# luigifreda/plvs

Measured on AMD Instinct MI355X. Metric: Mvoxels/sec TSDF integrate (chisel 5 cm / 5 m, 640x480 RGB-D), higher is better.
Workload: dtype f32; 1 GPU; configs[2] stand-in, STREAMING: see DESIGN.md 4.1 / 4.6; mode=order-free (fixed-point sums; sdf / weight within tolerance), longest_voxel_run=25008, parallelism=chunk-hash shard x1

## Files before the change

### plvs_amd/csrc/tsdf_walk.hpp

```cpp
#pragma once
#include <hip/hip_runtime.h>

#include <cstdint>

#include "tsdf_chisel_core.hpp"
#include "tsdf_directory.hpp"
#include "tsdf_tiles.hpp"
#include "tsdf_walk_table.hpp"

namespace {

using namespace plvs::chisel;
using plvs::tsdf::cloud_of;
using plvs::tsdf::tile_span;
using plvs::tsdf::tile_span_tables;
using plvs::tsdf::TileSpan;
using plvs::tsdf::kCoordBias;
using plvs::tsdf::kErrCoordRange;
using plvs::tsdf::kErrDirectoryMiss;
using plvs::tsdf::kErrPoolFull;
using plvs::tsdf::home_bucket;
using plvs::tsdf::next_bucket;

constexpr int kWalkRays = 512;
constexpr int kMaskWords = kWalkRays / 32;
#ifndef PLVS_WALK_ENTRIES
#define PLVS_WALK_ENTRIES 4096
#endif
constexpr int kWalkEntries = PLVS_WALK_ENTRIES;
constexpr int kWalkLimit = kWalkEntries * 7 / 8;
constexpr int kWalkWindow = kWalkLimit / 2;
constexpr int kWalkChunks = 64;
constexpr uint32_t kErrScratch = 8u;

#ifdef PLVS_WALK_PROF
__device__ unsigned long long g_walk_prof[16];
__device__ unsigned long long g_apply_items[8192][4];
#define WALK_PROF_BEGIN()                                         \
  long long prof_t = (long long)clock64();                        \
  unsigned long long prof_acc[9] = {0, 0, 0, 0, 0, 0, 0, 0, 0}
#define WALK_PROF(k)                                               \
  do {                                                             \
    const long long now = (long long)clock64();                    \
    prof_acc[k] += (unsigned long long)(now - prof_t);             \
    prof_t = now;                                                  \
  } while (0)
#define WALK_PROF_END()                                            \
  do {                                                             \
    if (threadIdx.x == 0)                                          \
      for (int k = 0; k < 9; ++k) atomicAdd(&g_walk_prof[k], prof_acc[k]); \
  } while (0)
#else
#define WALK_PROF_BEGIN() do {} while (0)
#define WALK_PROF(k) do {} while (0)
#define WALK_PROF_END() do {} while (0)
#endif

struct WalkCounters {
  unsigned long long total_visits;
  uint32_t err;
  uint32_t num_heads;
  uint32_t num_updated;
  uint32_t max_run;
  uint32_t num_desc;
  uint32_t run_need;
  uint32_t rec_top, seg_top;
  uint32_t ncold;
  uint32_t split_tiles;
  uint32_t num_parts;
  uint32_t num_multi;
  uint32_t ndeferred;
  uint32_t ndeferred2;
  uint32_t over_small;
  uint32_t skip;
  uint32_t collect_top;
  uint32_t collect_parts;
  uint32_t ndeferred3;
};

constexpr int kLogLen = 16;
constexpr int kSlabs = 8;
constexpr int kSlabVox = kChunkVox / kSlabs;

struct SubTile {
  uint16_t lo, hi;
  uint32_t vlo, vhi;
  int32_t cloud;
};

constexpr uint32_t kKeyEmpty = 0xFFFFFFFFu;
constexpr int kBuckets = kWalkEntries / 4;
constexpr int kOriginBias = 512;

constexpr int log2_of(int v) { return v <= 1 ? 0 : 1 + log2_of(v / 2); }
struct WalkShared {
  static constexpr int kEntries = kWalkEntries, kBucketCount = kWalkEntries / 4, kLogLen = ::kLogLen;
  alignas(16) uint32_t ekey[kWalkEntries];
  int32_t org[3];
  uint32_t cand[kWalkRays / 64];
  int32_t worg[kWalkRays / 64][3];
  uint32_t run_total, vis_total;
  uint32_t ccode[kWalkChunks];
  int32_t cslot[kWalkChunks];
  uint32_t ccnt[kWalkChunks * kSlabs];
  uint16_t cbase[kWalkChunks * kSlabs];
  uint32_t rbase;
  SubTile stack[16];
  int sp;
  uint32_t nent;
  uint32_t overflow;
  uint32_t wsum[kWalkRays / 64];
  uint32_t next, nrays;
};
template <int E>
struct FastShared {
  static constexpr int kEntries = E, kBucketCount = E / 4, kLogLen = E == 1536 ? ::kLogLen - 1 : ::kLogLen;
  static_assert(E % kWalkRays == 0 && E >= 1024, "every thread owns E / kWalkRays entries (and a bucket four)");
  alignas(16) uint32_t ekey[E];
  uint32_t cand[kWalkRays / 64];
  int32_t worg[kWalkRays / 64][3];
  uint32_t run_total, vis_total;
  uint32_t ccode[kWalkChunks];
  int32_t cslot[kWalkChunks];
  uint32_t ccnt[kWalkChunks * kSlabs];
  uint16_t cbase[kWalkChunks * kSlabs];
  uint32_t rcnt[kWalkChunks * kSlabs];
  uint16_t rcbase[kWalkChunks * kSlabs];
  uint32_t any_cold;
  uint32_t nent, overflow;
};


__device__ __forceinline__ bool rel_key(int vx, int vy, int vz, int ox, int oy, int oz, uint32_t* key) {
  const uint32_t dx = (uint32_t)(vx - ox), dy = (uint32_t)(vy - oy), dz = (uint32_t)(vz - oz);
  *key = dx | (dy << 10) | (dz << 20);
  return ((dx | dy | dz) >> 10) == 0u;
}
__device__ __forceinline__ int origin_of(int v) { return (v - kOriginBias) & ~15; }
constexpr uint32_t kChunkCodeMask = 0x3F0FC3F0u;
__device__ __forceinline__ uint32_t chunk_code(uint32_t key) { return key & kChunkCodeMask; }
__device__ __forceinline__ uint32_t voxel_in_chunk(uint32_t key) {
  return (key & 15u) | ((key >> 6) & 0xF0u) | ((key >> 12) & 0xF00u);
}
__device__ __forceinline__ void chunk_of_code(uint32_t code, int ox, int oy, int oz, int* cx, int* cy, int* cz) {
  *cx = (ox >> 4) + (int)((code >> 4) & 63u);
  *cy = (oy >> 4) + (int)((code >> 14) & 63u);
  *cz = (oz >> 4) + (int)((code >> 24) & 63u);
}
constexpr uint32_t kKeyMul = plvs::tsdf::kTableKeyMul, kKeyMulInv = plvs::tsdf::kTableKeyMulInv;
__device__ __forceinline__ uint32_t table_key(uint32_t key) { return key * kKeyMul; }
__device__ __forceinline__ uint32_t voxel_key(uint32_t tkey) { return tkey * kKeyMulInv; }
template <class SH>
__device__ __forceinline__ uint32_t key_bucket(uint32_t tkey) { return home_bucket<SH::kBucketCount>(tkey); }

__device__ __forceinline__ uint32_t wave_scan_incl(uint32_t x) {
  x += (uint32_t)__builtin_amdgcn_update_dpp(0, (int)x, 0x111, 0xf, 0xf, false);
  x += (uint32_t)__builtin_amdgcn_update_dpp(0, (int)x, 0x112, 0xf, 0xf, false);
  x += (uint32_t)__builtin_amdgcn_update_dpp(0, (int)x, 0x114, 0xf, 0xf, false);
  x += (uint32_t)__builtin_amdgcn_update_dpp(0, (int)x, 0x118, 0xf, 0xf, false);
  x += (uint32_t)__builtin_amdgcn_update_dpp(0, (int)x, 0x142, 0xa, 0xf, false);
  x += (uint32_t)__builtin_amdgcn_update_dpp(0, (int)x, 0x143, 0xc, 0xf, false);
  return x;
}
__device__ __forceinline__ uint32_t wave_sum(uint32_t x) {
  return (uint32_t)__builtin_amdgcn_readlane((int)wave_scan_incl(x), 63);
}

__device__ __forceinline__ int bucket_match(const uint4 k4, uint32_t want) {
  const bool c0 = k4.x == want, c1 = k4.y == want, c2 = k4.z == want, c3 = k4.w == want;
  const int j = c3 ? 3 : (c2 ? 2 : (c1 ? 1 : 0));
  return (c0 | c1 | c2 | c3) ? j : -1;
}

constexpr int kProbeCap = plvs::tsdf::kTableProbeCap;
template <class SH>
__device__ __forceinline__ int table_find_or_insert(SH& S, uint32_t key ) {
  uint32_t b = key_bucket<SH>(key);
  for (int probe = 0; probe < kProbeCap; ++probe) {
    const uint4 k4 = *reinterpret_cast<const uint4*>(&S.ekey[4 * b]);
    const int j = bucket_match(k4, key);
    if (j >= 0) return (int)(4 * b) + j;
    const int je = bucket_match(k4, kKeyEmpty);
    if (je >= 0) {
      const uint32_t old = atomicCAS(&S.ekey[4 * b + je], kKeyEmpty, key);
      if (old == kKeyEmpty || old == key) return (int)(4 * b) + je;
      continue;
    }
    b = next_bucket<SH::kBucketCount>(b);
  }
  S.overflow = 1u;
  return -1;
}
template <class SH>
__device__ __forceinline__ int table_find(const SH& S, uint32_t key) {
  uint32_t b = key_bucket<SH>(key);
  for (int probe = 0; probe < SH::kBucketCount; ++probe) {
    const int j = bucket_match(*reinterpret_cast<const uint4*>(&S.ekey[4 * b]), key);
    if (j >= 0) return (int)(4 * b) + j;
    b = next_bucket<SH::kBucketCount>(b);
  }
  return -1;
}

__device__ __forceinline__ float sqrt_rn_normal(float x) {
  const float s = __builtin_amdgcn_sqrtf(x);
  const float sm = __uint_as_float(__float_as_uint(s) - 1u), sp = __uint_as_float(__float_as_uint(s) + 1u);
  const float rm = fmaf(-sm, s, x), rp = fmaf(-sp, s, x);
  float r = (rm <= 0.0f) ? sm : s;
  r = (rp > 0.0f) ? sp : r;
  return r;
}
__device__ __forceinline__ float div_rn_normal(float a, float b) {
// ... 1 lines not shown
  const float y = fmaf(fmaf(-b, y0, 1.0f), y0, y0);
  const float q = a * y;
  return fmaf(fmaf(-q, b, a), y, q);
}
__device__ __forceinline__ float signed_dist_fast(const Pose& pose, float depth, float c0, float c1, float c2) {
  float cc[3];
  xform(pose.Ri, pose.ti, c0, c1, c2, cc);
  const float n2 = sqnorm3(cc[0], cc[1], cc[2]);
  const bool plain = !(n2 >= 0x1p-80f && n2 <= 0x1p80f) || !(fabsf(cc[2]) >= 0x1p-40f && fabsf(cc[2]) <= 0x1p40f);
  if (__builtin_expect(plain, 0)) return sqrtf(n2) * (depth / cc[2] - 1);
  return sqrt_rn_normal(n2) * (div_rn_normal(depth, cc[2]) - 1);
}
__device__ __forceinline__ float uniform_f(float x) {
  return __int_as_float(__builtin_amdgcn_readfirstlane(__float_as_int(x)));
}
struct LeanRay {
  float A[9], b[3];
  float tau_in, tau_out;
};
__device__ __forceinline__ void lean_ray(const Params& P, const Pose& pose, const Ray& ray, LeanRay* L) {
#pragma unroll
  for (int k = 0; k < 9; ++k) L->A[k] = uniform_f(pose.Ri[k] * P.resolution);
#pragma unroll
  for (int k = 0; k < 3; ++k)
    L->b[k] = uniform_f(fmaf(pose.Ri[3 * k], P.half_voxel, fmaf(pose.Ri[3 * k + 1], P.half_voxel, fmaf(pose.Ri[3 * k + 2], P.half_voxel, pose.ti[k]))));
  const float mx = (ray.start[0] + ray.end[0]) * (0.5f * P.resolution) - pose.t[0];
  const float my = (ray.start[1] + ray.end[1]) * (0.5f * P.resolution) - pose.t[1];
  const float mz = (ray.start[2] + ray.end[2]) * (0.5f * P.resolution) - pose.t[2];
  const float obl2 = fmaxf(sqnorm3(mx, my, mz) / (ray.depth * ray.depth), 1.0f);
  float ext = 0.0f;
#pragma unroll
  for (int k = 0; k < 3; ++k) ext = fmaxf(ext, fmaxf(fabsf(ray.start[k]), fabsf(ray.end[k])));
  const float m = fabsf(pose.ti[0]) + fabsf(pose.ti[1]) + fabsf(pose.ti[2]) + 3.0f * (ext + 4.0f) * P.resolution + ray.depth + 1.0f;
  const float band = m * obl2 * 0x1p-19f;
  L->tau_in = ray.truncation - band;
  L->tau_out = ray.truncation + band;
}
__device__ __forceinline__ float lean_u(const LeanRay& L, float depth, float fx, float fy, float fz) {
  const float c0 = fmaf(L.A[0], fx, fmaf(L.A[1], fy, fmaf(L.A[2], fz, L.b[0])));
  const float c1 = fmaf(L.A[3], fx, fmaf(L.A[4], fy, fmaf(L.A[5], fz, L.b[1])));
  const float c2 = fmaf(L.A[6], fx, fmaf(L.A[7], fy, fmaf(L.A[8], fz, L.b[2])));
  const float n2 = fmaf(c0, c0, fmaf(c1, c1, c2 * c2));
  return __builtin_amdgcn_sqrtf(n2) * ((depth - c2) * __builtin_amdgcn_rcpf(c2));
}
__device__ __forceinline__ bool two_tier_visit(const Params& P, const Pose& pose, const Ray& ray, const LeanRay& L, float fx,
                                               float fy, float fz, float* u) {
  *u = lean_u(L, ray.depth, fx, fy, fz);
  const float au = fabsf(*u);
  bool in = au < L.tau_in;
  if (__builtin_expect(!in && au < L.tau_out, 0)) {
    const float c0 = fx * P.resolution + P.half_voxel, c1 = fy * P.resolution + P.half_voxel,
                c2 = fz * P.resolution + P.half_voxel;
    *u = signed_dist_fast(pose, ray.depth, c0, c1, c2);
    in = fabsf(*u) < ray.truncation;
  }
  return in;
}

template <class OnVisit>
__device__ __forceinline__ uint32_t walk_one(const Params& P, const Pose& pose, const Ray& ray, uint32_t vlo,
                                             uint32_t vhi, OnVisit&& on_visit) {
  RayCursor cur;
  OwnerCache owner;
  LeanRay L;
  lean_ray(P, pose, ray, &L);
  ray_begin(ray, &cur);
  int vx, vy, vz;
  uint32_t nv = 0;
  bool go = true;
  while (go && nv < vhi && ray_next(&cur, &vx, &vy, &vz)) {
    float u = 0.0f;
    const bool ok = chunk_owned(P, vx >> 4, vy >> 4, vz >> 4, &owner) &&
                    two_tier_visit(P, pose, ray, L, (float)vx, (float)vy, (float)vz, &u);
    if (ok && nv >= vlo) go = on_visit(nv - vlo, vx, vy, vz, u);
    nv += ok ? 1u : 0u;
  }
  return nv;
}

__device__ __forceinline__ int lean_reach(const Ray& ray) {
  const float maxDist = sqnorm3(ray.end[0] - ray.start[0], ray.end[1] - ray.start[1], ray.end[2] - ray.start[2]);
  return (int)(__builtin_amdgcn_sqrtf(maxDist)) + 3;
}
template <bool kAcc, bool kRuns, bool kRayOfVp, class SH>
__device__ __forceinline__ uint32_t walk_lean(const Params& P, const Pose& pose, const Ray& ray, SH& S, int ox, int oy,
                                              int oz, int tid, float wu_scaled, uint32_t q_w, int32_t* e_wuu,
                                              unsigned long long* e_wc, uint32_t* e_last, uint16_t* vlog, uint32_t rid) {
  RayCursor cur;
  ray_begin(ray, &cur);
  if (cur.done) return 0u;
  LeanRay L;
  lean_ray(P, pose, ray, &L);
  uint32_t key = table_key((uint32_t)(cur.x - ox) | ((uint32_t)(cur.y - oy) << 10) | ((uint32_t)(cur.z - oz) << 20));
  const uint32_t endkey = table_key((uint32_t)(cur.endX - ox) | ((uint32_t)(cur.endY - oy) << 10) | ((uint32_t)(cur.endZ - oz) << 20));
  const uint32_t kx = table_key((uint32_t)cur.stepX), ky = table_key((uint32_t)cur.stepY << 10), kz = table_key((uint32_t)cur.stepZ << 20);
  float fx = (float)cur.x, fy = (float)cur.y, fz = (float)cur.z;
  const float sfx = (float)cur.stepX, sfy = (float)cur.stepY, sfz = (float)cur.stepZ;
  float tmx = cur.tMaxX, tmy = cur.tMaxY, tmz = cur.tMaxZ;
  const float tdx = cur.stepX ? cur.tDeltaX : 0.0f, tdy = cur.stepY ? cur.tDeltaY : 0.0f, tdz = cur.stepZ ? cur.tDeltaZ : 0.0f;
  static_assert(kWalkRays * sizeof(uint16_t) == 1024, "the count is the offset >> 10");
  uint32_t vp = (uint32_t)tid * (uint32_t)sizeof(uint16_t);
  for (int guard = 0; guard < kRayStepGuard; ++guard) {
    const float d = sqnorm3(fx - cur.sx, fy - cur.sy, fz - cur.sz);
    const bool stop = (d > cur.maxDist) || (key == endkey);
    float u;
    if (two_tier_visit(P, pose, ray, L, fx, fy, fz, &u)) {
      int e;
      {
        const uint32_t b = key_bucket<SH>(key);
        const uint4 k4 = *reinterpret_cast<const uint4*>(&S.ekey[4 * b]);
        const int j = bucket_match(k4, key);
        if (j >= 0) {
          e = (int)(4 * b) + j;
        } else {
          const int je = bucket_match(k4, kKeyEmpty);
          uint32_t old = 0u;
          if (je >= 0) old = atomicCAS(&S.ekey[4 * b + je], kKeyEmpty, key);
          e = (je >= 0 && (old == kKeyEmpty || old == key)) ? (int)(4 * b) + je : table_find_or_insert(S, key);
        }
      }
      if (__builtin_expect(e < 0, 0)) break;
      if (kRuns && vp < (uint32_t)(SH::kLogLen * kWalkRays * sizeof(uint16_t)))
        *reinterpret_cast<uint16_t*>(reinterpret_cast<char*>(vlog) + vp) = (uint16_t)e;
      if (kAcc) {
        atomicAdd(&e_wuu[e], __float2int_rn(wu_scaled * u));
        atomicAdd(&e_wc[e], (1ull << 32) | (unsigned long long)q_w);
        atomicMax(&e_last[e], kRayOfVp ? (vp >> 1) & (uint32_t)(kWalkRays - 1) : rid);
      }
      vp += (uint32_t)(kWalkRays * sizeof(uint16_t));
    }
    if (stop) break;
    const bool x_lt_y = tmx < tmy, x_lt_z = tmx < tmz, y_lt_z = tmy < tmz;
    const bool go_x = x_lt_y && x_lt_z, go_y = !x_lt_y && y_lt_z;
    const float mx = go_x ? 1.0f : 0.0f, my = go_y ? 1.0f : 0.0f, mz = (go_x || go_y) ? 0.0f : 1.0f;
    fx = fmaf(mx, sfx, fx);
    fy = fmaf(my, sfy, fy);
    fz = fmaf(mz, sfz, fz);
    tmx = fmaf(mx, tdx, tmx);
    tmy = fmaf(my, tdy, tmy);
    tmz = fmaf(mz, tdz, tmz);
    key += go_x ? kx : (go_y ? ky : kz);
  }
  return vp >> 10;
}

constexpr int kGridTileW = 32, kGridTileH = kWalkRays / kGridTileW;
static_assert(kGridTileW == 32 && kGridTileH == kMaskWords, "one mask word per grid row of a tile");
struct GridSrc {
  const float* depth;
  const float* cam;
  unsigned long long image_stride;
  uint32_t pitch;
  uint32_t step, gw, gh;
  uint32_t ntx, nty;
  uint32_t key_bits;
  double min_depth, max_depth;
  unsigned long long bgr_image_stride;
  uint32_t bgr_pitch;
  float inv_ntx, inv_nty;
};
struct GridTile {
  uint32_t cloud, row0, col0;
};
__device__ __forceinline__ uint32_t fast_div(uint32_t x, uint32_t d, float inv) {
  if (x >= (1u << 24)) return x / d;
  uint32_t q = (uint32_t)((float)x * inv);
  const int32_t r = (int32_t)(x - q * d);
  q = r < 0 ? q - 1u : ((uint32_t)r >= d ? q + 1u : q);
  return q;
}
__device__ __forceinline__ uint32_t grid_band(const GridSrc& g, uint32_t gtile) { return fast_div(gtile, g.ntx, g.inv_ntx); }
__device__ __forceinline__ GridTile grid_tile_of_band(const GridSrc& g, uint32_t gtile, uint32_t band) {
  const uint32_t c = fast_div(band, g.nty, g.inv_nty);
  return GridTile{c, (band - c * g.nty) * (uint32_t)kGridTileH, (gtile - band * g.ntx) * (uint32_t)kGridTileW};
}
__device__ __forceinline__ GridTile grid_tile(const GridSrc& g, uint32_t gtile) {
  return grid_tile_of_band(g, gtile, grid_band(g, gtile));
}
__device__ __forceinline__ bool grid_point(const GridSrc& g, const GridTile& t, uint32_t rid, float* x, float* y, float* z) {
  const uint32_t m = t.row0 + rid / (uint32_t)kGridTileW, n = t.col0 + rid % (uint32_t)kGridTileW;
  if (m >= g.gh || n >= g.gw) return false;
  const float d = g.depth[(size_t)t.cloud * g.image_stride + (size_t)(m * g.step) * g.pitch + n * g.step];
  if (!(((double)d > g.min_depth) && ((double)d < g.max_depth))) return false;
  const float2 c = reinterpret_cast<const float2*>(g.cam)[m * g.gw + n];
  *x = c.x * d;
  *y = c.y * d;
  *z = d;
  return true;
}
typedef float GridFloat2 __attribute__((ext_vector_type(2)));
__device__ __forceinline__ GridSrc grid_fetch(const GridSrc* __restrict__ gp) {
  GridSrc g{};
  g.depth = gp->depth; g.cam = gp->cam; g.image_stride = gp->image_stride; g.pitch = gp->pitch; g.step = gp->step;
  g.gw = gp->gw; g.gh = gp->gh; g.ntx = gp->ntx; g.nty = gp->nty; g.min_depth = gp->min_depth; g.max_depth = gp->max_depth;
  g.inv_ntx = gp->inv_ntx; g.inv_nty = gp->inv_nty;
  asm volatile("" ::"s"(g.depth), "s"(g.cam), "s"(g.image_stride), "s"(g.pitch), "s"(g.step), "s"(g.gw), "s"(g.gh), "s"(g.ntx),
               "s"(g.nty), "s"(g.min_depth), "s"(g.max_depth), "s"(g.inv_ntx), "s"(g.inv_nty));
  return g;
}
__device__ __forceinline__ bool grid_pixel_load(const GridSrc& g, const GridTile& t, uint32_t rid, float* d, GridFloat2* c) {
  const uint32_t m = t.row0 + rid / (uint32_t)kGridTileW, n = t.col0 + rid % (uint32_t)kGridTileW;
  if (m >= g.gh || n >= g.gw) return false;
  const auto* depth = (const __attribute__((address_space(1))) float*)(uintptr_t)g.depth;
  const auto* cam = (const __attribute__((address_space(1))) GridFloat2*)(uintptr_t)g.cam;
  *d = depth[(size_t)t.cloud * g.image_stride + (size_t)(m * g.step) * g.pitch + n * g.step];
  *c = cam[m * g.gw + n];
  return true;
// ... 532 lines not shown
    }
    for (uint32_t r0 = 0; fits_runs && r0 < nruns; r0 += kMaskCap) {
      __syncthreads();
#pragma unroll
      for (int k = 0; k < kMaskCap * kMaskWords / kWalkRays; ++k) raw[tid + k * kWalkRays] = 0u;
      __syncthreads();
      if (walks && nmine) {
        const uint32_t logged = min(nmine, (uint32_t)kLogLen);
        for (uint32_t k = 0; k < logged; ++k) {
          const uint32_t m = (uint32_t)e_midx[vlog[k * kWalkRays + tid]] - r0;
          if (m < (uint32_t)kMaskCap) atomicOr(&raw[m * kMaskWords + (tid >> 5)], 1u << (tid & 31));
        }
        if (nmine > (uint32_t)kLogLen) {
          walk_one(P, pose, ray, st.vlo, st.vhi, [&](uint32_t k, int vx, int vy, int vz, float) {
            if (k >= (uint32_t)kLogLen) {
              uint32_t key;
              const int e = rel_key(vx, vy, vz, fox, foy, foz, &key) ? table_find(S, table_key(key)) : -1;
              const uint32_t m = e >= 0 ? (uint32_t)e_midx[e] - r0 : 0xFFFFFFFFu;
              if (m < (uint32_t)kMaskCap) atomicOr(&raw[m * kMaskWords + (tid >> 5)], 1u << (tid & 31));
            }
            return true;
          });
        }
      }
      __syncthreads();
#pragma unroll
      for (int k = 0; k < kPer; ++k) {
        const uint32_t m = (uint32_t)e_midx[tid + k * kWalkRays];
        if (m == 0xFFFFu || m < r0 || m >= r0 + (uint32_t)kMaskCap) continue;
        const size_t d = ((size_t)tile << runs.r1_log2) + emitted + m;
        runs.dkey[d] = vkey[k];
        const uint32_t* mk = raw + (m - r0) * kMaskWords;
        uint4* dst = reinterpret_cast<uint4*>(runs.masks + d * kMaskWords);
#pragma unroll
        for (int q = 0; q < kMaskWords / 4; ++q) dst[q] = make_uint4(mk[4 * q], mk[4 * q + 1], mk[4 * q + 2], mk[4 * q + 3]);
      }
    }
    __syncthreads();
    if (tid == 0) S.run_total = emitted + nruns;
    WALK_PROF(7);
    if (single && !was_split) break;
  }

#pragma unroll
  for (int off = 32; off > 0; off >>= 1) my_visits += (uint32_t)__shfl_xor((int)my_visits, off);
  if (lane == 0 && my_visits) atomicAdd(&S.vis_total, my_visits);
  __syncthreads();
  if (tid == 0) {
    if (kRuns) runs.run_cnt[tile] = min(S.run_total, 1u << runs.r1_log2);
    if (kAcc) {
      out.tile_visits[tile] = S.vis_total;
      if (flushes == 0) out.seg_cnt[tile] = 0;
    }
    if (was_split) atomicAdd(&ctr->split_tiles, 1u);
  }
  WALK_PROF(8);
  WALK_PROF_END();
  }
}

constexpr int walk_fast_waves(int E) { return E > 2048 ? 2 : (E > 1536 ? 4 : 6); }
constexpr int kFastEntriesSmall = 1536;
template <int E, bool kGrid>
__device__ __forceinline__ void walk_fast_tile(
    const Params& P, float scale_u, float scale_w, const float* __restrict__ xyz, int npoints,
    const int32_t* __restrict__ offsets, int nclouds, const Pose* __restrict__ poses, const Directory& dir,
    int32_t* __restrict__ num_chunks, WalkCounters* __restrict__ ctr, const uint32_t* __restrict__ rgbw,
    const uint32_t* __restrict__ sat, const AccOut& out, const RunOut& runs, const TileMap& tmap, uint32_t rec_stride,
    uint32_t* __restrict__ deferred, uint32_t* __restrict__ ndeferred, const uint32_t tile, const bool listed_other,
    const GridSrc* __restrict__ grid_arg) {
  const GridSrc* __restrict__ const grid = kGrid ? grid_arg : nullptr;
  constexpr int kPer = E / kWalkRays;
  constexpr int kLimit = E * 7 / 8;
  constexpr int kMaskCapE = E / 4;
  constexpr int kLogLen = FastShared<E>::kLogLen;
  static_assert(kMaskCapE * kMaskWords % kWalkRays == 0, "the mask area is cleared by whole rounds of the tile's threads");
  __shared__ FastShared<E> S;
  __shared__ uint32_t raw[4 * E];
  __shared__ uint16_t vlog[kLogLen * kWalkRays];
  static_assert(offsetof(FastShared<E>, cbase) == offsetof(FastShared<E>, ccnt) + sizeof(S.ccnt), "cbase follows ccnt");
  constexpr bool kMidxOverlay = sizeof(S.ccnt) + sizeof(S.cbase) >= E * sizeof(uint16_t);
  __shared__ uint16_t e_midx_own[kMidxOverlay ? 1 : E];
  uint16_t* const e_midx = kMidxOverlay ? reinterpret_cast<uint16_t*>(S.ccnt) : e_midx_own;
  int32_t* const e_wuu = reinterpret_cast<int32_t*>(raw);
  unsigned long long* const e_wc = reinterpret_cast<unsigned long long*>(raw + E);
  uint32_t* const e_last = raw + 3 * E;
  const int tid = threadIdx.x, lane = tid & 63, wid = tid >> 6;
  const uint32_t gtile = tmap.tile_of(tile);
  const GridSrc gs = kGrid ? grid_fetch(grid_arg) : GridSrc{};
  const GridTile gt = kGrid ? grid_tile(gs, gtile) : GridTile{0u, 0u, 0u};
  const TileSpan span = grid ? TileSpan{(int)gt.cloud, 0u, (uint32_t)kWalkRays}
                      : tmap.tables ? tile_span_tables(offsets, nclouds, gtile, kWalkRays)
                                    : tile_span(offsets, nclouds, gtile, kWalkRays);
  const uint32_t first = span.first, nrays = span.nrays;
  const int cloud = span.cloud;
  bool defer = P.shard_count > 1 || listed_other;
  WALK_PROF_BEGIN();
  uint32_t nv = 0;
  uint32_t rid = (uint32_t)threadIdx.x;
  bool walks = false;
  int ox = 0, oy = 0, oz = 0;
  if (!defer) {
    const Pose& pose = poses[cloud];
    float gd = 0.0f, pR[9], pt[3];
    GridFloat2 gc = {0.0f, 0.0f};
    bool gin = false;
    if (kGrid) {
      gin = grid_pixel_load(gs, gt, rid, &gd, &gc);
#pragma unroll
      for (int k = 0; k < 9; ++k) pR[k] = pose.R[k];
#pragma unroll
      for (int k = 0; k < 3; ++k) pt[k] = pose.t[k];
    }
    subtile_reset(S, tid);
#pragma unroll
    for (int k = 0; k < kWalkChunks * kSlabs / kWalkRays; ++k) S.rcnt[tid + k * kWalkRays] = 0u;
#pragma unroll
    for (int k = 0; k < 4 * kPer; ++k) raw[tid + k * kWalkRays] = 0u;
    if (tid == 0) {
      S.run_total = 0;
      S.vis_total = 0;
      S.any_cold = 0;
    }
    Ray ray;
    if (kGrid) {
      asm volatile("" ::"s"(pR[0]), "s"(pR[1]), "s"(pR[2]), "s"(pR[3]), "s"(pR[4]), "s"(pR[5]), "s"(pR[6]), "s"(pR[7]), "s"(pR[8]),
                   "s"(pt[0]), "s"(pt[1]), "s"(pt[2]));
      Pose cw{};
#pragma unroll
      for (int k = 0; k < 9; ++k) cw.R[k] = pR[k];
#pragma unroll
      for (int k = 0; k < 3; ++k) cw.t[k] = pt[k];
      walks = gin && grid_depth_ok(gs, gd) && ray_of_point(P, cw, gc.x * gd, gc.y * gd, gd, &ray, &ctr->err);
    } else {
      walks = (uint32_t)tid < nrays && tile_ray_src(P, xyz, grid, gt, pose, first, rid, &ray, &ctr->err);
    }
    const float wu = walks ? P.weight / (2.0f * ray.truncation) : 0.0f;
    {
      const unsigned long long wm = __ballot(walks);
      if (lane == 0) S.cand[wid] = wm ? 1u : 0u;
      if (wm && lane == __ffsll((long long)wm) - 1)
        for (int k = 0; k < 3; ++k) S.worg[wid][k] = origin_of((int)floorf(ray.start[k]));
    }
    WALK_PROF(0);
    __syncthreads();
    WALK_PROF(1);
    {
      int w0 = 0;
#pragma unroll
      for (int w = kWalkRays / 64 - 1; w >= 0; --w) w0 = S.cand[w] ? w : w0;
      ox = S.worg[w0][0]; oy = S.worg[w0][1]; oz = S.worg[w0][2];
      uint32_t anyc = 0;
#pragma unroll
      for (int w = 0; w < kWalkRays / 64; ++w) anyc |= S.cand[w];
      if (anyc == 0u) {
        if (tid == 0) {
          out.seg_cnt[tile] = 0;
          runs.run_cnt[tile] = 0;
          out.tile_visits[tile] = 0;
        }
        return;
      }
    }
    bool fits = false;
    if (walks) {
      const int reach = lean_reach(ray);
      const int rx = (int)floorf(ray.start[0]) - ox, ry = (int)floorf(ray.start[1]) - oy, rz = (int)floorf(ray.start[2]) - oz;
      fits = min(min(rx, ry), rz) - reach >= 0 && max(max(rx, ry), rz) + reach <= 1023;
      if (!fits) S.overflow = 1u;
    }
    if (fits) {
      nv = walk_lean<true, true, true>(P, pose, ray, S, ox, oy, oz, tid, wu * scale_u, (uint32_t)__float2int_rn(wu * scale_w), e_wuu,
                                 e_wc, e_last, vlog, rid);
    }
  }
  uint32_t ekey[kPer];
  WALK_PROF(2);
  if (!defer) {
    __syncthreads();
    WALK_PROF(3);
#pragma unroll
    for (int k = 0; k < kPer; ++k) {
      ekey[k] = S.ekey[tid + k * kWalkRays];
      if (ekey[k] != kKeyEmpty) ekey[k] = voxel_key(ekey[k]);
    }
    uint32_t wave_n = 0;
#pragma unroll
    for (int k = 0; k < kPer; ++k) wave_n += (uint32_t)__popcll(__ballot(ekey[k] != kKeyEmpty));
    if (lane == 0 && wave_n) atomicAdd(&S.nent, wave_n);
  } else {
#pragma unroll
    for (int k = 0; k < kPer; ++k) ekey[k] = kKeyEmpty;
  }
  int ci[kPer];
  uint32_t rank[kPer], rrank[kPer], vkey[kPer], elast[kPer];
  unsigned long long ewc[kPer];
  uint32_t need = 0;
  bool multi = false;
#pragma unroll
  for (int k = 0; k < kPer; ++k) {
    ci[k] = -2;
    rank[k] = 0;
    rrank[k] = 0;
    vkey[k] = 0xFFFFFFFFu;
    elast[k] = 0;
    ewc[k] = 0;
  }
  if (!defer) {
#pragma unroll
    for (int k = 0; k < kPer; ++k) {
      if (ekey[k] == kKeyEmpty) continue;
      bool won;
      ci[k] = chunk_cache_insert(S, chunk_code(ekey[k]), &won);
      if (ci[k] < 0) {
        S.overflow = 1u;
        continue;
      }
      int slot = S.cslot[ci[k]];
      if (slot < 0) {
        int cx, cy, cz;
        chunk_of_code(chunk_code(ekey[k]), ox, oy, oz, &cx, &cy, &cz);
        slot = dir_find_or_insert_hit(dir, cx, cy, cz, num_chunks, &ctr->err);
        if (slot >= 0) S.cslot[ci[k]] = slot;
      }
      if (slot < 0) continue;
      vkey[k] = (uint32_t)slot * (uint32_t)kChunkVox + voxel_in_chunk(ekey[k]);
    }
    uint32_t cw[kPer];
#pragma unroll
    for (int k = 0; k < kPer; ++k) {
      cw[k] = 0u;
      if (vkey[k] != 0xFFFFFFFFu) cw[k] = sat ? sat[vkey[k] >> 5] : rgbw[vkey[k]];
    }
#pragma unroll
    for (int k = 0; k < kPer; ++k) {
      if (vkey[k] == 0xFFFFFFFFu) continue;
      const uint32_t vid = vkey[k] % (uint32_t)kChunkVox;
      ewc[k] = e_wc[tid + k * kWalkRays];
      elast[k] = e_last[tid + k * kWalkRays];
      rank[k] = atomicAdd(&S.ccnt[ci[k] * kSlabs + (int)(vid / kSlabVox)], 1u);
    }
#pragma unroll
    for (int k = 0; k < kPer; ++k) {
      if (vkey[k] == 0xFFFFFFFFu) continue;
      const bool cold = sat ? ((cw[k] >> (vkey[k] & 31u)) & 1u) == 0u : (cw[k] >> 24) < 254u;
      if (cold) {
        need |= 1u << k;
        multi = multi || (uint32_t)(ewc[k] >> 32) > 1u;
        rrank[k] = atomicAdd(&S.rcnt[ci[k] * kSlabs + (int)((vkey[k] % (uint32_t)kChunkVox) / kSlabVox)], 1u);
      }
    }
  }
  WALK_PROF(4);
  if (need) S.any_cold = 1u;
  const bool any_multi = __syncthreads_or(multi ? 1 : 0) != 0;
  const bool any_cold = S.any_cold != 0u;
  WALK_PROF(5);
  const bool too_many = !defer && S.nent > (uint32_t)kLimit;
  if (E == 2048 && tid == 0 && !defer && S.nent > (uint32_t)(kFastEntriesSmall * 7 / 8)) atomicAdd(&ctr->over_small, 1u);
  if (!defer) defer = S.overflow != 0 || too_many;
  if (defer) {
    if (tid == 0) {
      out.seg_cnt[tile] = 0;
      runs.run_cnt[tile] = 0;
      out.tile_visits[tile] = 0;
      deferred[atomicAdd(ndeferred, 1u)] = tile | (too_many ? 0x80000000u : 0u);
    }
    return;
  }
  {
    const uint32_t v = wave_sum(nv);
    if (lane == 0 && v) atomicAdd(&S.vis_total, v);
  }
  const uint32_t rbase = tile * rec_stride;
  uint32_t nruns;
  uint32_t ticket = 0, ticket_sg = 0xFFFFFFFFu;
  {
    uint32_t sub[kSlabs], c = 0, rsub[kSlabs], rc = 0;
#pragma unroll
    for (int s = 0; s < kSlabs; ++s) {
      sub[s] = c;
      c += S.ccnt[lane * kSlabs + s];
      rsub[s] = 0;
    }
    uint32_t rinc = 0;
    nruns = 0;
    if (any_cold) {
#pragma unroll
      for (int s = 0; s < kSlabs; ++s) {
        rsub[s] = rc;
        rc += S.rcnt[lane * kSlabs + s];
      }
      rinc = wave_scan_incl(rc);
      nruns = (uint32_t)__builtin_amdgcn_readlane((int)rinc, 63);
#pragma unroll
      for (int s = 0; s < kSlabs; ++s) S.rcbase[lane * kSlabs + s] = (uint16_t)(rinc - rc + rsub[s]);
    }
    const uint32_t both = wave_scan_incl(c | (c ? 1u << 16 : 0u));
    const uint32_t inc = both & 0xFFFFu, sinc = both >> 16;
#pragma unroll
    for (int s = 0; s < kSlabs; ++s) S.cbase[lane * kSlabs + s] = (uint16_t)(inc - c + sub[s]);
    if (wid == 0) {
      const uint32_t stot = (uint32_t)__builtin_amdgcn_readlane((int)sinc, 63);
      if (lane == 0) out.seg_cnt[tile] = stot;
      if (c) {
        const uint32_t sg = tile * (uint32_t)kWalkChunks + sinc - 1u;
        if (out.chunk_nseg) {
          ticket = atomicAdd(&out.chunk_nseg[S.cslot[lane]], 1u);
          ticket_sg = sg;
        }
        out.seg[2 * (size_t)sg] = make_uint4((uint32_t)S.cslot[lane], rbase + inc - c, c, gtile);
        out.seg[2 * (size_t)sg + 1] = pack_suboffsets(sub);
        if (runs.rseg) {
          runs.rseg[2 * (size_t)sg] = make_uint4((tile << runs.r1_log2) + rinc - rc, rc, 0u, 0u);
          runs.rseg[2 * (size_t)sg + 1] = pack_suboffsets(rsub);
        }
      }
    }
  }
#pragma unroll
  for (int k = 0; k < kPer; ++k) {
    if (vkey[k] == 0xFFFFFFFFu) continue;
    const uint32_t vid = vkey[k] % (uint32_t)kChunkVox;
    const uint4 r = make_uint4(vid | ((uint32_t)(ewc[k] >> 32) << 12),
                               grid ? grid_order_key(*grid, gt, elast[k]) : first + elast[k],
                               (uint32_t)e_wuu[tid + k * kWalkRays], (uint32_t)ewc[k]);
    out.rec[rbase + S.cbase[ci[k] * kSlabs + (int)(vid / kSlabVox)] + rank[k]] = r;
  }
  WALK_PROF(6);
  const bool fits_runs = nruns <= (1u << runs.r1_log2);
  if (!fits_runs && tid == 0) {
    atomicOr(&ctr->err, kErrScratch);
    atomicMax(&ctr->run_need, nruns);
  }
  uint32_t mrun[kPer];
#pragma unroll
  for (int k = 0; k < kPer; ++k)
    mrun[k] = (need & (1u << k)) ? (uint32_t)S.rcbase[ci[k] * kSlabs + (int)((vkey[k] % (uint32_t)kChunkVox) / kSlabVox)] + rrank[k] : 0xFFFFu;
  if (!any_multi) {
#pragma unroll
    for (int k = 0; k < kPer; ++k) {
      if (!(need & (1u << k)) || !fits_runs) continue;
      const size_t d = ((size_t)tile << runs.r1_log2) + mrun[k];
      runs.dkey[d] = vkey[k];
      uint4* dst = reinterpret_cast<uint4*>(runs.masks + d * kMaskWords);
      const uint32_t word = elast[k] >> 5, bit = 1u << (elast[k] & 31u);
#pragma unroll
      for (int q = 0; q < kMaskWords / 4; ++q)
        dst[q] = make_uint4(word == 4u * q ? bit : 0u, word == 4u * q + 1u ? bit : 0u, word == 4u * q + 2u ? bit : 0u,
                            word == 4u * q + 3u ? bit : 0u);
    }
  } else {
    __syncthreads();
#pragma unroll
    for (int k = 0; k < kPer; ++k) e_midx[tid + k * kWalkRays] = (uint16_t)mrun[k];
    for (uint32_t r0 = 0; fits_runs && r0 < nruns; r0 += kMaskCapE) {
      __syncthreads();
#pragma unroll
      for (int k = 0; k < kMaskCapE * kMaskWords / kWalkRays; ++k) raw[tid + k * kWalkRays] = 0u;
      __syncthreads();
      if (nv) {
        const uint32_t logged = min(nv, (uint32_t)kLogLen);
        for (uint32_t k = 0; k < logged; ++k) {
          const uint32_t m = (uint32_t)e_midx[vlog[k * kWalkRays + tid]] - r0;
          if (m < (uint32_t)kMaskCapE) atomicOr(&raw[m * kMaskWords + (rid >> 5)], 1u << (rid & 31));
        }
        if (nv > (uint32_t)kLogLen) {
          const Pose& pose = poses[cloud];
          Ray ray;
          if (tile_ray_src(P, xyz, grid, gt, pose, first, rid, &ray, &ctr->err))
            walk_one(P, pose, ray, 0u, 0xFFFFFFFFu, [&](uint32_t k, int vx, int vy, int vz, float) {
              if (k >= (uint32_t)kLogLen) {
                uint32_t key;
                const int e = rel_key(vx, vy, vz, ox, oy, oz, &key) ? table_find(S, table_key(key)) : -1;
                const uint32_t m = e >= 0 ? (uint32_t)e_midx[e] - r0 : 0xFFFFFFFFu;
                if (m < (uint32_t)kMaskCapE) atomicOr(&raw[m * kMaskWords + (rid >> 5)], 1u << (rid & 31));
              }
              return true;
            });
        }
      }
      __syncthreads();
#pragma unroll
      for (int k = 0; k < kPer; ++k) {
        const uint32_t m = (uint32_t)e_midx[tid + k * kWalkRays];
        if (m == 0xFFFFu || m < r0 || m >= r0 + (uint32_t)kMaskCapE) continue;
        const size_t d = ((size_t)tile << runs.r1_log2) + m;
        runs.dkey[d] = vkey[k];
        const uint32_t* mk = raw + (m - r0) * kMaskWords;
        uint4* dst = reinterpret_cast<uint4*>(runs.masks + d * kMaskWords);
#pragma unroll
        for (int q = 0; q < kMaskWords / 4; ++q) dst[q] = make_uint4(mk[4 * q], mk[4 * q + 1], mk[4 * q + 2], mk[4 * q + 3]);
      }
    }
  }
  if (tid == 0) S.run_total = nruns;
  WALK_PROF(7);
  __syncthreads();
  WALK_PROF(8);
  WALK_PROF_END();
  if (tid == 0) {
    runs.run_cnt[tile] = min(S.run_total, 1u << runs.r1_log2);
    out.tile_visits[tile] = S.vis_total;
  }
  if (ticket_sg != 0xFFFFFFFFu) out.seg_ticket[ticket_sg] = ticket;
}

template <int E, bool kGrid = false, bool kList = false>
__global__ __launch_bounds__(kWalkRays, walk_fast_waves(E)) void walk_fast(
    Params P, float scale_u, float scale_w, const float* __restrict__ xyz, int npoints,
    const int32_t* __restrict__ offsets, int nclouds, const Pose* __restrict__ poses, Directory dir,
    int32_t* __restrict__ num_chunks, WalkCounters* __restrict__ ctr, const uint32_t* __restrict__ rgbw,
    const uint32_t* __restrict__ sat, AccOut out, RunOut runs, TileMap tmap, uint32_t rec_stride,
    const uint32_t* __restrict__ tile_list, const uint32_t* __restrict__ ntile_list, uint32_t* __restrict__ deferred,
    uint32_t* __restrict__ ndeferred, const GridSrc* __restrict__ grid) {
  if constexpr (!kList) {
    walk_fast_tile<E, kGrid>(P, scale_u, scale_w, xyz, npoints, offsets, nclouds, poses, dir, num_chunks, ctr, rgbw, sat, out, runs,
                      tmap, rec_stride, deferred, ndeferred, blockIdx.x, false, grid);
  } else {
    const uint32_t nlist = *ntile_list;
    for (uint32_t lb = blockIdx.x; lb < nlist; lb += gridDim.x) {
      const uint32_t e = tile_list[lb];
      walk_fast_tile<E, kGrid>(P, scale_u, scale_w, xyz, npoints, offsets, nclouds, poses, dir, num_chunks, ctr, rgbw, sat, out,
                        runs, tmap, rec_stride, deferred, ndeferred, e & 0x7FFFFFFFu, (e >> 31) == 0u, grid);
      __syncthreads();
    }
  }
}

constexpr int kSegSpan = 1024;
constexpr uint32_t kPartSegs = 256;
constexpr uint32_t kPartMin = 512;
constexpr int kSegTable = 512;
template <bool kScatter>
__global__ __launch_bounds__(256) void seg_pass(const uint4* __restrict__ seg, uint32_t seg_cap, uint32_t ntiles,
                                                const uint32_t* __restrict__ seg_cnt, uint32_t* __restrict__ chunk_nseg,
                                                const uint32_t* __restrict__ chunk_off, uint32_t* __restrict__ chunk_fill,
                                                uint4* __restrict__ sorted, const WalkCounters* __restrict__ ctr) {
  __shared__ uint32_t hkey[kSegTable], hcnt[kSegTable], hbase[kSegTable];
  const int tid = threadIdx.x;
  const uint32_t own = ntiles * (uint32_t)kWalkChunks;
  const uint32_t n = min(own + ctr->seg_top, seg_cap);
  for (int k = tid; k < kSegTable; k += 256) {
    hkey[k] = 0xFFFFFFFFu;
    hcnt[k] = 0;
  }
  __syncthreads();
  constexpr int kSpan = kSegSpan, kPer = kSpan / 256;
  int ent[kPer];
  uint32_t rnk[kPer], slot[kPer];
#pragma unroll
  for (int q = 0; q < kPer; ++q) {
    const uint32_t j = blockIdx.x * (uint32_t)kSpan + (uint32_t)(q * 256 + tid);
    ent[q] = -2;
    if (j >= n || (j < own && (j % kWalkChunks) >= seg_cnt[j / kWalkChunks])) continue;
    slot[q] = seg[2 * (size_t)j].x;
    uint32_t h = (slot[q] * 2654435761u) >> (32 - 9);
    ent[q] = -1;
    for (int probe = 0; probe < kSegTable; ++probe) {
      uint32_t cur = hkey[h];
      if (cur == 0xFFFFFFFFu) cur = atomicCAS(&hkey[h], 0xFFFFFFFFu, slot[q]);
      if (cur == 0xFFFFFFFFu || cur == slot[q]) {
        ent[q] = (int)h;
        break;
      }
      h = (h + 1) & (kSegTable - 1);
    }
    if (ent[q] >= 0) rnk[q] = atomicAdd(&hcnt[ent[q]], 1u);
  }
  __syncthreads();
  for (int k = tid; k < kSegTable; k += 256) {
    if (hkey[k] == 0xFFFFFFFFu) continue;
    if (kScatter) hbase[k] = chunk_off[hkey[k]] + atomicAdd(&chunk_fill[hkey[k]], hcnt[k]);
    else atomicAdd(&chunk_nseg[hkey[k]], hcnt[k]);
  }
// ... 1453 lines not shown
```

Before: 92440 Mvoxels/s.

## Pack per-entry visit accumulators and spill overflowing visit logs to shared list

```diff
diff --git a/plvs_amd/csrc/tsdf_walk.hpp b/plvs_amd/csrc/tsdf_walk.hpp
--- a/plvs_amd/csrc/tsdf_walk.hpp
+++ b/plvs_amd/csrc/tsdf_walk.hpp
@@ -7,6 +7,7 @@
 #include "tsdf_directory.hpp"
 #include "tsdf_tiles.hpp"
 #include "tsdf_walk_table.hpp"
+#include "tsdf_walk_visit.hpp"
 
 namespace {
 
@@ -95,6 +96,7 @@
 constexpr int log2_of(int v) { return v <= 1 ? 0 : 1 + log2_of(v / 2); }
 struct WalkShared {
   static constexpr int kEntries = kWalkEntries, kBucketCount = kWalkEntries / 4, kLogLen = ::kLogLen;
+  static constexpr int kSpillCap = -1;
   alignas(16) uint32_t ekey[kWalkEntries];
   int32_t org[3];
   uint32_t cand[kWalkRays / 64];
@@ -128,6 +130,9 @@
   uint16_t rcbase[kWalkChunks * kSlabs];
   uint32_t any_cold;
   uint32_t nent, overflow;
+  static constexpr int kSpillCap = 128;
+  uint32_t nspill;
+  uint32_t spill[kSpillCap];
 };
 
 
@@ -295,7 +300,7 @@
   const float maxDist = sqnorm3(ray.end[0] - ray.start[0], ray.end[1] - ray.start[1], ray.end[2] - ray.start[2]);
   return (int)(__builtin_amdgcn_sqrtf(maxDist)) + 3;
 }
-template <bool kAcc, bool kRuns, bool kRayOfVp, class SH>
+template <bool kAcc, bool kRuns, bool kRayOfVp, bool kVisitWords = false, class SH>
 __device__ __forceinline__ uint32_t walk_lean(const Params& P, const Pose& pose, const Ray& ray, SH& S, int ox, int oy,
                                               int oz, int tid, float wu_scaled, uint32_t q_w, int32_t* e_wuu,
                                               unsigned long long* e_wc, uint32_t* e_last, uint16_t* vlog, uint32_t rid) {
@@ -333,9 +338,17 @@
         }
       }
       if (__builtin_expect(e < 0, 0)) break;
-      if (kRuns && vp < (uint32_t)(SH::kLogLen * kWalkRays * sizeof(uint16_t)))
+      if (kRuns && vp < (uint32_t)(SH::kLogLen * kWalkRays * sizeof(uint16_t))) {
         *reinterpret_cast<uint16_t*>(reinterpret_cast<char*>(vlog) + vp) = (uint16_t)e;
-      if (kAcc) {
+      } else if constexpr (kRuns && kRayOfVp && SH::kSpillCap >= 0) {
+        const uint32_t n = atomicAdd(&S.nspill, 1u);
+        if (n < (uint32_t)SH::kSpillCap) S.spill[n] = (((vp >> 1) & (uint32_t)(kWalkRays - 1)) << 16) | (uint32_t)e;
+      }
+      if (kAcc && kVisitWords) {
+        static_assert(!kVisitWords || kRayOfVp, "the visit words are the lean tiles': the ray is the thread");
+        atomicAdd(&e_wc[e], plvs::tsdf::visit_sums_word(__float2int_rn(wu_scaled * u), q_w));
+        atomicAdd(&e_last[e], plvs::tsdf::visit_count_word((vp >> 1) & (uint32_t)(kWalkRays - 1)));
+      } else if (kAcc) {
         atomicAdd(&e_wuu[e], __float2int_rn(wu_scaled * u));
         atomicAdd(&e_wc[e], (1ull << 32) | (unsigned long long)q_w);
         atomicMax(&e_last[e], kRayOfVp ? (vp >> 1) & (uint32_t)(kWalkRays - 1) : rid);
@@ -1034,9 +1047,11 @@
   constexpr bool kMidxOverlay = sizeof(S.ccnt) + sizeof(S.cbase) >= E * sizeof(uint16_t);
   __shared__ uint16_t e_midx_own[kMidxOverlay ? 1 : E];
   uint16_t* const e_midx = kMidxOverlay ? reinterpret_cast<uint16_t*>(S.ccnt) : e_midx_own;
+  static_assert(plvs::tsdf::visit_words_hold<kWalkRays>(), "count and ray sum of a whole tile fit the count word");
   int32_t* const e_wuu = reinterpret_cast<int32_t*>(raw);
-  unsigned long long* const e_wc = reinterpret_cast<unsigned long long*>(raw + E);
-  uint32_t* const e_last = raw + 3 * E;
+  unsigned long long* const e_wc = reinterpret_cast<unsigned long long*>(kGrid ? raw : raw + E);
+  uint32_t* const e_last = raw + (kGrid ? 2 : 3) * E;
+  constexpr int kAccWords = kGrid ? 3 : 4;
   const int tid = threadIdx.x, lane = tid & 63, wid = tid >> 6;
   const uint32_t gtile = tmap.tile_of(tile);
   const GridSrc gs = kGrid ? grid_fetch(grid_arg) : GridSrc{};
@@ -1068,11 +1083,12 @@
 #pragma unroll
     for (int k = 0; k < kWalkChunks * kSlabs / kWalkRays; ++k) S.rcnt[tid + k * kWalkRays] = 0u;
 #pragma unroll
-    for (int k = 0; k < 4 * kPer; ++k) raw[tid + k * kWalkRays] = 0u;
+    for (int k = 0; k < kAccWords * kPer; ++k) raw[tid + k * kWalkRays] = 0u;
     if (tid == 0) {
       S.run_total = 0;
       S.vis_total = 0;
       S.any_cold = 0;
+      S.nspill = 0;
     }
     Ray ray;
     if (kGrid) {
@@ -1122,8 +1138,8 @@
       if (!fits) S.overflow = 1u;
     }
     if (fits) {
-      nv = walk_lean<true, true, true>(P, pose, ray, S, ox, oy, oz, tid, wu * scale_u, (uint32_t)__float2int_rn(wu * scale_w), e_wuu,
-                                 e_wc, e_last, vlog, rid);
+      nv = walk_lean<true, true, true, kGrid>(P, pose, ray, S, ox, oy, oz, tid, wu * scale_u, (uint32_t)__float2int_rn(wu * scale_w),
+                                              e_wuu, e_wc, e_last, vlog, rid);
     }
   }
   uint32_t ekey[kPer];
@@ -1188,7 +1204,7 @@
     for (int k = 0; k < kPer; ++k) {
       if (vkey[k] == 0xFFFFFFFFu) continue;
       const uint32_t vid = vkey[k] % (uint32_t)kChunkVox;
-      ewc[k] = e_wc[tid + k * kWalkRays];
+      if (!kGrid) ewc[k] = e_wc[tid + k * kWalkRays];
       elast[k] = e_last[tid + k * kWalkRays];
       rank[k] = atomicAdd(&S.ccnt[ci[k] * kSlabs + (int)(vid / kSlabVox)], 1u);
     }
@@ -1198,7 +1214,7 @@
       const bool cold = sat ? ((cw[k] >> (vkey[k] & 31u)) & 1u) == 0u : (cw[k] >> 24) < 254u;
       if (cold) {
         need |= 1u << k;
-        multi = multi || (uint32_t)(ewc[k] >> 32) > 1u;
+        multi = multi || (kGrid ? plvs::tsdf::visit_count(elast[k]) : (uint32_t)(ewc[k] >> 32)) > 1u;
         rrank[k] = atomicAdd(&S.rcnt[ci[k] * kSlabs + (int)((vkey[k] % (uint32_t)kChunkVox) / kSlabVox)], 1u);
       }
     }
@@ -1270,13 +1286,20 @@
       }
     }
   }
+  const uint32_t tile_key = kGrid ? grid_order_key(*grid, gt, 0u) : 0u;
 #pragma unroll
   for (int k = 0; k < kPer; ++k) {
     if (vkey[k] == 0xFFFFFFFFu) continue;
     const uint32_t vid = vkey[k] % (uint32_t)kChunkVox;
-    const uint4 r = make_uint4(vid | ((uint32_t)(ewc[k] >> 32) << 12),
-                               grid ? grid_order_key(*grid, gt, elast[k]) : first + elast[k],
-                               (uint32_t)e_wuu[tid + k * kWalkRays], (uint32_t)ewc[k]);
+    uint4 r;
+    if (kGrid) {
+      const unsigned long long sums = e_wc[tid + k * kWalkRays];
+      r = make_uint4(vid | (plvs::tsdf::visit_count(elast[k]) << 12), tile_key, plvs::tsdf::visit_sum_wuu(sums),
+                     plvs::tsdf::visit_sum_w(sums));
+    } else {
+      r = make_uint4(vid | ((uint32_t)(ewc[k] >> 32) << 12), first + elast[k], (uint32_t)e_wuu[tid + k * kWalkRays],
+                     (uint32_t)ewc[k]);
+    }
     out.rec[rbase + S.cbase[ci[k] * kSlabs + (int)(vid / kSlabVox)] + rank[k]] = r;
   }
   WALK_PROF(6);
@@ -1296,7 +1319,8 @@
       const size_t d = ((size_t)tile << runs.r1_log2) + mrun[k];
       runs.dkey[d] = vkey[k];
       uint4* dst = reinterpret_cast<uint4*>(runs.masks + d * kMaskWords);
-      const uint32_t word = elast[k] >> 5, bit = 1u << (elast[k] & 31u);
+      const uint32_t one = kGrid ? plvs::tsdf::visit_ray_sum(elast[k]) : elast[k];
+      const uint32_t word = one >> 5, bit = 1u << (one & 31u);
 #pragma unroll
       for (int q = 0; q < kMaskWords / 4; ++q)
         dst[q] = make_uint4(word == 4u * q ? bit : 0u, word == 4u * q + 1u ? bit : 0u, word == 4u * q + 2u ? bit : 0u,
@@ -1306,31 +1330,24 @@
     __syncthreads();
 #pragma unroll
     for (int k = 0; k < kPer; ++k) e_midx[tid + k * kWalkRays] = (uint16_t)mrun[k];
+    constexpr uint32_t kSpillCap = (uint32_t)FastShared<E>::kSpillCap;
+    static_assert(kSpillCap <= (uint32_t)kWalkRays, "a thread per listed visit");
+    const uint32_t nspill = S.nspill;
     for (uint32_t r0 = 0; fits_runs && r0 < nruns; r0 += kMaskCapE) {
       __syncthreads();
-#pragma unroll
-      for (int k = 0; k < kMaskCapE * kMaskWords / kWalkRays; ++k) raw[tid + k * kWalkRays] = 0u;
+      const uint32_t nclear = min(nruns - r0, (uint32_t)kMaskCapE) * (uint32_t)kMaskWords;
+#pragma unroll 1
+      for (uint32_t i = (uint32_t)tid; i < nclear; i += (uint32_t)kWalkRays) raw[i] = 0u;
       __syncthreads();
-      if (nv) {
-        const uint32_t logged = min(nv, (uint32_t)kLogLen);
-        for (uint32_t k = 0; k < logged; ++k) {
-          const uint32_t m = (uint32_t)e_midx[vlog[k * kWalkRays + tid]] - r0;
-          if (m < (uint32_t)kMaskCapE) atomicOr(&raw[m * kMaskWords + (rid >> 5)], 1u << (rid & 31));
-        }
-        if (nv > (uint32_t)kLogLen) {
-          const Pose& pose = poses[cloud];
-          Ray ray;
-          if (tile_ray_src(P, xyz, grid, gt, pose, first, rid, &ray, &ctr->err))
-            walk_one(P, pose, ray, 0u, 0xFFFFFFFFu, [&](uint32_t k, int vx, int vy, int vz, float) {
-              if (k >= (uint32_t)kLogLen) {
-                uint32_t key;
-                const int e = rel_key(vx, vy, vz, ox, oy, oz, &key) ? table_find(S, table_key(key)) : -1;
-                const uint32_t m = e >= 0 ? (uint32_t)e_midx[e] - r0 : 0xFFFFFFFFu;
-                if (m < (uint32_t)kMaskCapE) atomicOr(&raw[m * kMaskWords + (rid >> 5)], 1u << (rid & 31));
-              }
-              return true;
-            });
-        }
+      const uint32_t logged = min(nv, (uint32_t)kLogLen);
+      for (uint32_t k = 0; k < logged; ++k) {
+        const uint32_t m = (uint32_t)e_midx[vlog[k * kWalkRays + tid]] - r0;
+        if (m < (uint32_t)kMaskCapE) atomicOr(&raw[m * kMaskWords + (rid >> 5)], 1u << (rid & 31));
+      }
+      if ((uint32_t)tid < nspill && nspill <= kSpillCap) {
+        const uint32_t w = S.spill[tid], sr = w >> 16;
+        const uint32_t m = (uint32_t)e_midx[w & 0xFFFFu] - r0;
+        if (m < (uint32_t)kMaskCapE) atomicOr(&raw[m * kMaskWords + (sr >> 5)], 1u << (sr & 31));
       }
       __syncthreads();
 #pragma unroll
@@ -1343,6 +1360,24 @@
         uint4* dst = reinterpret_cast<uint4*>(runs.masks + d * kMaskWords);
 #pragma unroll
         for (int q = 0; q < kMaskWords / 4; ++q) dst[q] = make_uint4(mk[4 * q], mk[4 * q + 1], mk[4 * q + 2], mk[4 * q + 3]);
+      }
+    }
+    if (fits_runs && nspill > kSpillCap) {
+      __syncthreads();
+      if (nv > (uint32_t)kLogLen) {
+        const Pose& pose = poses[cloud];
+        Ray ray;
+        if (tile_ray_src(P, xyz, grid, gt, pose, first, rid, &ray, &ctr->err))
+          walk_one(P, pose, ray, 0u, 0xFFFFFFFFu, [&](uint32_t k, int vx, int vy, int vz, float) {
+            if (k >= (uint32_t)kLogLen) {
+              uint32_t key;
+              const int e = rel_key(vx, vy, vz, ox, oy, oz, &key) ? table_find(S, table_key(key)) : -1;
+              const uint32_t m = e >= 0 ? (uint32_t)e_midx[e] : 0xFFFFu;
+              if (m != 0xFFFFu)
+                atomicOr(&runs.masks[(((size_t)tile << runs.r1_log2) + m) * kMaskWords + (rid >> 5)], 1u << (rid & 31));
+            }
+            return true;
+          });
       }
     }
   }
diff --git a/plvs_amd/csrc/tsdf_walk_visit.hpp b/plvs_amd/csrc/tsdf_walk_visit.hpp
--- /dev/null
+++ b/plvs_amd/csrc/tsdf_walk_visit.hpp
@@ -0,0 +1,34 @@
+#pragma once
+
+#include <cstdint>
+
+#if defined(__HIPCC__)
+#define PLVS_VISIT_FN __host__ __device__ __forceinline__
+#else
+#define PLVS_VISIT_FN inline
+#endif
+
+namespace plvs {
+namespace tsdf {
+
+constexpr int kVisitCountBits = 10;
+constexpr uint32_t kVisitCountMask = (1u << kVisitCountBits) - 1u;
+
+template <int kRays>
+constexpr bool visit_words_hold() {
+  return (uint64_t)kRays <= (uint64_t)kVisitCountMask &&
+         ((uint64_t)kRays * (uint64_t)(kRays - 1) / 2) < (1ull << (32 - kVisitCountBits));
+}
+
+PLVS_VISIT_FN unsigned long long visit_sums_word(int32_t wuu, uint32_t q_w) {
+  return ((unsigned long long)(long long)wuu << 32) + (unsigned long long)q_w;
+}
+PLVS_VISIT_FN uint32_t visit_count_word(uint32_t ray) { return (ray << kVisitCountBits) | 1u; }
+
+PLVS_VISIT_FN uint32_t visit_sum_wuu(unsigned long long sums) { return (uint32_t)(sums >> 32); }
+PLVS_VISIT_FN uint32_t visit_sum_w(unsigned long long sums) { return (uint32_t)sums; }
+PLVS_VISIT_FN uint32_t visit_count(uint32_t word) { return word & kVisitCountMask; }
+PLVS_VISIT_FN uint32_t visit_ray_sum(uint32_t word) { return word >> kVisitCountBits; }
+
+}
+}
```

Result: faster. 95880 Mvoxels/s, median of 6 (+3.7%).
